# hahnyuan/PTQ4ViT

Measured on AMD Instinct MI355X. Metric: calibration throughput (wrapped modules calibrated per second), ViT-B/224 W8A8, 32 calibration images, higher is better.
Workload: dtype int8

## Files before the change

### include/ptq4vit_hip_debug.h

```cpp
#ifndef PTQ4VIT_HIP_DEBUG_H
#define PTQ4VIT_HIP_DEBUG_H

#include <stdint.h>

#ifdef __cplusplus
extern "C" {
#endif

int p4v_debug_set_variant(int variant, int force_generic);
int p4v_debug_set_tuning(int key, int value);
int p4v_debug_bound_totals(float* out, int64_t capacity, int64_t* count);
int p4v_debug_topk_rows(const float* d_mass, int segs, int n, int k, int32_t* d_idx, void* stream);
int p4v_debug_pack_dual(const float* d_x, long rows, long cols, long cols_padded, int sos, int lo, int hi, int qmax,
                        const float* d_scale, float const_scale, int8_t* d_q1, int8_t* d_q2, void* stream);
int p4v_debug_pack_cands(const float* d_x, long rows, long cols, long rows_padded, long cols_padded, int layout, int lo, int hi,
                         const float* d_scales, int n_cands, const int* d_crange, const unsigned char* d_done, int live_max,
                         int general, int8_t* d_q, void* stream);
int p4v_debug_gather_im2col(int batch, int in_channels, int height, int width, int kernel_h, int kernel_w, int stride_h, int stride_w,
                            int pad_h, int pad_w, int dil_h, int dil_w, const float* d_x, const int32_t* d_idx, int k, float* d_dst,
                            void* stream);
int p4v_debug_prep_epi6(const float* d_o, const float* d_wt, const float* d_bias, long o_ss, long o_ts, int sr, int tr,
                        int bias_on_t, int wt_mode, int transposed, float* d_e, void* stream);

#ifdef __cplusplus
}
#endif
#endif
```

### ptq4vit_amd/_lib.py

```python
import ctypes as C
import os

_HERE = os.path.dirname(os.path.abspath(__file__))
LIB_PATH = os.environ.get("P4V_LIB") or os.path.join(_HERE, "csrc", "libptq4vit_hip.so")

METRICS = {
    "L1_norm": 0,
    "L2_norm": 1,
    "linear_weighted_L2_norm": 2,
    "square_weighted_L2_norm": 3,
    "hessian": 4,
    "cosine": 5,
}


class LinearDesc(C.Structure):
    _fields_ = [(n, C.c_int32) for n in (
        "batch", "tokens", "in_features", "out_features", "n_V", "n_H", "n_a", "w_bit", "a_bit", "metric",
        "eq_n", "search_round", "twin_postgelu", "init_layerwise", "has_bias", "reserved")]


class MatMulDesc(C.Structure):
    _fields_ = ([(n, C.c_int32) for n in ("batch", "heads", "M", "K", "N")] + [("_pad0", C.c_int32)] +
                [("a_stride", C.c_int64 * 4), ("b_stride", C.c_int64 * 4)] +
# ... 43 lines not shown
                ("scale1_stride", C.c_int64 * 4), ("scale1_div", C.c_int32 * 4),
                ("scale2_stride", C.c_int64 * 4), ("scale2_div", C.c_int32 * 4),
                ("scale2_const", C.c_float),
                ("mode", C.c_int32), ("lo1", C.c_int32), ("hi1", C.c_int32), ("lo2", C.c_int32), ("hi2", C.c_int32),
                ("qmax", C.c_int32), ("reserved", C.c_int32)]


class GroupJob(C.Structure):
    _fields_ = [("kind", C.c_int32), ("status", C.c_int32), ("desc", C.c_void_p), ("inp", C.c_void_p * 5), ("mult", C.c_void_p),
                ("out", C.c_void_p * 3), ("workspace", C.c_void_p), ("workspace_bytes", C.c_size_t)]


JOB_LINEAR, JOB_MATMUL, JOB_CONV, JOB_MATMUL_BLOCKS = 0, 1, 2, 3
PLANE_SYM, PLANE_SOS_HI, PLANE_SOS_LO, PLANE_TWIN = 1, 2, 3, 4
EXPORT_SYM_I8, EXPORT_SYM_F32, EXPORT_GELU_U8, EXPORT_SOS_U8 = 0, 1, 2, 3


EXPORTS = [
    "p4v_version", "p4v_last_error",
    "p4v_linear_workspace_bytes", "p4v_linear_calibrate",
    "p4v_matmul_workspace_bytes", "p4v_matmul_calibrate",
    "p4v_matmul_blocks_workspace_bytes", "p4v_matmul_blocks_calibrate", "p4v_amax_init_matmul_blocks",
    "p4v_matmul_blocks_search", "p4v_matmul_blocks_quant_forward",
    "p4v_conv_workspace_bytes", "p4v_conv_calibrate",
    "p4v_calibrate_group", "p4v_launch_counters",
    "p4v_linear_quant_forward", "p4v_matmul_quant_forward",
    "p4v_amax_init_linear", "p4v_linear_search_w", "p4v_linear_search_a",
    "p4v_amax_init_matmul", "p4v_matmul_search_A", "p4v_sos_search_split", "p4v_matmul_search_B",
    "p4v_amax_init_conv", "p4v_conv_search_w_channelwise", "p4v_conv_search_w_layerwise", "p4v_conv_search_a",
    "p4v_score_argmax_gather",
    "p4v_quantize_i8", "p4v_pack_plane_i8", "p4v_fake_quant", "p4v_export_quantize", "p4v_multi_copy",
    "p4v_stats_enable", "p4v_stats_reset", "p4v_stats_get", "p4v_stats_launches", "p4v_prune_counters",
    "p4v_debug_set_variant", "p4v_debug_set_tuning", "p4v_debug_bound_totals", "p4v_debug_topk_rows", "p4v_debug_pack_dual", "p4v_debug_prep_epi6",
    "p4v_debug_pack_cands", "p4v_debug_gather_im2col",
]

_lib = None


def load():
    global _lib
    if _lib is not None:
        return _lib
    if not os.path.exists(LIB_PATH):
        raise RuntimeError(
            f"ptq4vit_amd: HIP extension {LIB_PATH} is missing -- build it with "
            "`python -c 'import __graft_entry__ as g; g.build()'` (hipcc --offload-arch=gfx950). "
            "There is no CPU fallback for the calibration path.")
    import torch
    lib = C.CDLL(LIB_PATH)
    vp, fp, ip = C.c_void_p, C.c_void_p, C.c_void_p
    lib.p4v_version.restype = C.c_int
    lib.p4v_last_error.restype = C.c_char_p
    lib.p4v_linear_workspace_bytes.restype = C.c_size_t
    lib.p4v_linear_workspace_bytes.argtypes = [C.POINTER(LinearDesc)]
    lib.p4v_linear_calibrate.restype = C.c_int
    lib.p4v_linear_calibrate.argtypes = [C.POINTER(LinearDesc), fp, fp, fp, fp, fp, fp, fp, fp, fp, ip, vp, C.c_size_t, vp]
    lib.p4v_matmul_workspace_bytes.restype = C.c_size_t
    lib.p4v_matmul_workspace_bytes.argtypes = [C.POINTER(MatMulDesc)]
    lib.p4v_matmul_calibrate.restype = C.c_int
    lib.p4v_matmul_calibrate.argtypes = [C.POINTER(MatMulDesc), fp, fp, fp, fp, fp, fp, fp, fp, fp, ip, vp, C.c_size_t, vp]
    MBD = C.POINTER(MatMulBlocksDesc)
    lib.p4v_matmul_blocks_workspace_bytes.restype = C.c_size_t
    lib.p4v_matmul_blocks_workspace_bytes.argtypes = [MBD]
    lib.p4v_matmul_blocks_calibrate.restype = C.c_int
    lib.p4v_matmul_blocks_calibrate.argtypes = [MBD, fp, fp, fp, fp, fp, fp, fp, fp, fp, ip, vp, C.c_size_t, vp]
    lib.p4v_amax_init_matmul_blocks.restype = C.c_int
# ... 18 lines not shown
            ("p4v_linear_search_a", [LD] + [fp] * 9 + [ip]),
            ("p4v_amax_init_matmul", [MD] + [fp] * 4),
            ("p4v_matmul_search_A", [MD] + [fp] * 8 + [ip]),
            ("p4v_sos_search_split", [MD] + [fp] * 7 + [ip]),
            ("p4v_matmul_search_B", [MD] + [fp] * 9 + [ip]),
            ("p4v_amax_init_conv", [CD] + [fp] * 4),
            ("p4v_conv_search_w_channelwise", [CD] + [fp] * 9 + [ip]),
            ("p4v_conv_search_w_layerwise", [CD] + [fp] * 9 + [ip]),
            ("p4v_conv_search_a", [CD] + [fp] * 9 + [ip])):
        fn = getattr(lib, name)
        fn.restype = C.c_int
        fn.argtypes = args + tail
    lib.p4v_score_argmax_gather.restype = C.c_int
    lib.p4v_score_argmax_gather.argtypes = [fp, C.c_int32, C.c_int32, fp, fp, ip, vp]
    lib.p4v_quantize_i8.restype = C.c_int
    lib.p4v_quantize_i8.argtypes = [fp, C.c_int64, C.c_int64, C.c_int64, fp, C.c_int64, C.c_int32, C.c_int32, vp, vp]
    lib.p4v_fake_quant.restype = C.c_int
    lib.p4v_fake_quant.argtypes = [fp, C.c_int64, C.c_int64, fp, C.c_int64, C.c_int32, C.c_int32, fp, vp]
    lib.p4v_pack_plane_i8.restype = C.c_int
    lib.p4v_pack_plane_i8.argtypes = [C.POINTER(PlaneDesc), fp, fp, vp, vp]
    lib.p4v_export_quantize.restype = C.c_int
    lib.p4v_export_quantize.argtypes = [C.POINTER(ExportDesc), fp, fp, fp, vp, vp]
    lib.p4v_multi_copy.restype = C.c_int
    lib.p4v_multi_copy.argtypes = [vp, C.c_int32, C.c_int64, C.c_int64, vp]
    lib.p4v_debug_topk_rows.restype = C.c_int
    lib.p4v_debug_topk_rows.argtypes = [vp, C.c_int, C.c_int, C.c_int, vp, vp]
    lib.p4v_debug_pack_dual.restype = C.c_int
    lib.p4v_debug_pack_dual.argtypes = [fp, C.c_long, C.c_long, C.c_long, C.c_int, C.c_int, C.c_int, C.c_int, fp, C.c_float, vp, vp, vp]
    lib.p4v_debug_pack_cands.restype = C.c_int
    lib.p4v_debug_pack_cands.argtypes = [fp, C.c_long, C.c_long, C.c_long, C.c_long, C.c_int, C.c_int, C.c_int, fp, C.c_int, vp, vp,
                                         C.c_int, C.c_int, vp, vp]
    lib.p4v_debug_gather_im2col.restype = C.c_int
    lib.p4v_debug_gather_im2col.argtypes = [C.c_int] * 12 + [fp, ip, C.c_int, fp, vp]
    lib.p4v_debug_prep_epi6.restype = C.c_int
    lib.p4v_debug_prep_epi6.argtypes = [fp, fp, fp, C.c_long, C.c_long, C.c_int, C.c_int, C.c_int, C.c_int, C.c_int, fp, vp]
    lib.p4v_debug_set_variant.restype = C.c_int
    lib.p4v_debug_set_variant.argtypes = [C.c_int, C.c_int]
    lib.p4v_debug_set_tuning.restype = C.c_int
    lib.p4v_debug_set_tuning.argtypes = [C.c_int, C.c_int]
    lib.p4v_debug_bound_totals.restype = C.c_int
    lib.p4v_debug_bound_totals.argtypes = [fp, C.c_int64, C.POINTER(C.c_int64)]
    lib.p4v_stats_enable.restype = C.c_int
    lib.p4v_stats_enable.argtypes = [C.c_int]
    lib.p4v_stats_reset.restype = C.c_int
    lib.p4v_stats_get.restype = C.c_int
    lib.p4v_stats_get.argtypes = [C.POINTER(KernelStats)]
    lib.p4v_stats_launches.restype = C.c_int
    lib.p4v_stats_launches.argtypes = [C.POINTER(LaunchRecord), C.c_int64, C.POINTER(C.c_int64)]
    lib.p4v_prune_counters.restype = C.c_int
    lib.p4v_prune_counters.argtypes = [C.POINTER(C.c_int64), C.c_int]
    lib.p4v_launch_counters.restype = C.c_int
    lib.p4v_launch_counters.argtypes = [C.POINTER(C.c_int64), C.c_int]
    lib.p4v_calibrate_group.restype = C.c_int
    lib.p4v_calibrate_group.argtypes = [C.POINTER(GroupJob), C.c_int32, vp, vp]
    _lib = lib
    return lib


def check(rc, what):
    if rc != 0:
        msg = load().p4v_last_error().decode("utf-8", "replace")
        if rc == -2:
            raise NotImplementedError(f"{what}: {msg}")
        raise RuntimeError(f"{what} failed (code {rc}): {msg}")


# ... 9 lines not shown
```

### ptq4vit_amd/csrc/p4v_api.hip

```cpp
#include <hip/hip_runtime.h>

#include <algorithm>
#include <atomic>
#include <climits>
#include <cstdarg>
#include <cstdio>
#include <condition_variable>
#include <cstring>
#include <deque>
#include <functional>
#include <thread>
#include <mutex>
#include <string>
#include <unordered_map>
#include <type_traits>
#include <vector>

#include "../../include/ptq4vit_hip.h"
#include "../../include/ptq4vit_hip_debug.h"
#include "p4v_kernels.h"

using namespace p4v;

namespace {
// ... 1721 lines not shown
            if (tune(TUNE_PRINT) > 0) fprintf(stderr, "[p4v] second tier: %d survivors of the %d-row slice -> %d of the %d-row slice (M %d N %d K %d)\n", nsurv, k, std::max(0, h[1] - h[0]), k2, ps.Mrows, ps.Ncols, ps.K);
            if (h[0] >= h[1]) return select_without_b2();
            rB = r3; rBblk = rblk3;
            hlo = h[0]; hhi = h[1];
            if (hm && ps.nj <= MIR_BLK) { for (int i = 0; i < 2 * ps.nj; ++i) hblk[i] = reinterpret_cast<volatile int*>(hm)[MIR_RB2 + i]; }
            else hblk_ok = false;
        }
    }
    Pass b2 = ps;
    b2.crange = rB; b2.crange_blk = rBblk; b2.scores_keep = S2; b2.no_select = true;
    b2.host_lo = hlo; b2.host_hi = hhi; b2.host_rblk = hblk_ok ? hblk : nullptr;
    b2.S1_pre = S1s; b2.S2_pre = S2s; b2.s_ready = true;
    g_stage = 3;
    { const int r_ = run_pass(c, b2); g_stage = 0; if (r_) return r_; }
    if (!c.dry) {
        if (virt) CHK(enqueue(c, KERN(MergeVirtParams, k_merge_virtual), dim3(cdiv(ps.nj, 64)), dim3(64), 0, MergeVirtParams{S2, SB, best_idx, ps.nj}));
        else CHK(enqueue(c, KERN(MergeParams, k_merge_scores), dim3(cdiv((long)tab, 256)), dim3(256), 0, MergeParams{S2, SB, (int)tab}));
        CHK(launch_pass_select(c, ps, S2));
    }
    c.ws.off = mark;
    return 0;
}

struct SosSplitJob {
    SliceCache* scache; bool host_sync_ok, prunable;
    SosSplitParams kp;
    int epi; double norm;
    const float* cands; float* split; float* A_iv; float aux_div;
    float* scores_out; int scores_out_ld; int32_t* best_out;
};
bool sos_split_ok(int M, int K, int N, bool cosm) {
    return !cosm && K <= 200 && M <= 256 && N <= 64 && !(g_variant & 131072);
}
template <int KS> int launch_sos_split_ks(Ctx& c, const SosSplitParams& kp, int epi, const StatInfo* si) {
    const dim3 grid(kp.halves, kp.Z), block(256);
    const size_t lds = (size_t)2 * KS * 64 * sizeof(float);
    P4V_EPI4(epi, return enqueue(c, KERN_T(SosSplitParams, k_sos_split, KS, E), grid, block, lds, kp, si))
}
SelectParams sos_select_params(const SosSplitJob& j, const float* scores) {
    return SelectParams{scores, j.kp.C, 1, j.cands, 1, 0, 0, j.split, 0, 0, j.A_iv, j.aux_div, j.scores_out, j.scores_out_ld, j.best_out};
}
int sos_sweep(Ctx& c, SosSplitJob& j, SosSplitParams kp, const int* crange, float* scores, int known_cands = -1) {
    const int slots = kp.halves * 4;
    float* part = c.ws.get<float>((size_t)kp.C * kp.Z * slots);
    if (!c.ws.ok()) return fail(P4V_ERR_WORKSPACE, "workspace too small: need >= %zu bytes", c.ws.off);
    kp.part = part; kp.crange = crange;
    if (!c.dry) {
        CHK(q_fill(c, part, 0, sizeof(float) * (size_t)kp.C * kp.Z * slots));
        const int KS = kp.K <= 64 ? 32 : kp.K <= 144 ? 72 : 100;
        double frac = 1.0;
        if (g_stat_on && crange && known_cands >= 0) frac = (double)known_cands / kp.C;
        else if (g_stat_on && crange) {
            int h[2] = {0, kp.C};
            CHK(q_d2h(c, h, crange, sizeof h));
            CHK(q_sync(c));
            frac = (double)std::max(0, std::min(h[1], kp.C) - std::max(h[0], 0)) / kp.C;
        }
        const StatInfo si{11, frac * (double)kp.Z * kp.halves * 128 * (2.0 * KS) * 64 * kp.C, frac * (double)kp.Z * kp.M * kp.K * kp.N * kp.C, g_stage, kp.halves, kp.Z,
                          4.0 * ((double)kp.Z * kp.M * kp.K + (double)kp.Z * kp.K * kp.N) + 8.0 * (double)kp.Z * kp.M * kp.N};
        const StatInfo* sp = &si;
        if (KS == 32) CHK(launch_sos_split_ks<32>(c, kp, j.epi, sp));
        else if (KS == 72) CHK(launch_sos_split_ks<72>(c, kp, j.epi, sp));
        else CHK(launch_sos_split_ks<100>(c, kp, j.epi, sp));
    }
    FinishParams fp{part, (long)kp.Z * slots, (long)slots, slots, 1, kp.Z, slots, kp.C, 0, 1, 1, j.norm, scores, crange};
    return launch_finish(c, fp);
}
int sos_select(Ctx& c, SosSplitJob& j, const float* scores) {
    return launch_select(c, sos_select_params(j, scores));
}
int run_sos_split(Ctx& c, SosSplitJob& j) {
    const size_t mark = c.ws.off;
    float* scores = c.ws.get<float>((size_t)j.kp.C);
    CHK(sos_sweep(c, j, j.kp, nullptr, scores));
    CHK(sos_select(c, j, scores));
    c.ws.off = mark;
    return 0;
}
int run_sos_split_pruned_impl(Ctx& c, SosSplitJob& j);
int run_sos_split_pruned(Ctx& c, SosSplitJob& j) {
    if (!(g_variant & 134217728) || c.dry || !j.split) return run_sos_split_pruned_impl(c, j);
    std::vector<float> keep;
    CHK(run_sos_split_pruned_impl(c, j));
    CHK(prune_crosscheck_begin(c, j.split, 1, keep));
    CHK(run_sos_split(c, j));
    return prune_crosscheck_end(c, j.split, 1, keep, "split search");
}
int run_sos_split_pruned_impl(Ctx& c, SosSplitJob& j) {
    const SosSplitParams& kp = j.kp;
    const int k = 16;
    if (!j.prunable || !j.scache || j.scores_out || j.best_out || (g_variant & 4194304) || kp.M < 64 || j.scache->loose) {
        PRUNE_COUNT((!j.prunable || !j.scache || j.scores_out || j.best_out || (g_variant & 4194304)) ? 3 : 2);
        return run_sos_split(c, j);
    }
    SliceGeo geo{false, kp.Z, kp.M, k, kp.N, kp.K, kp.O, (kp.wt_mode == 1 ? kp.G : nullptr), kp.wt_mode, (long)kp.N, kp.A, kp.a_r, kp.a_k,
                 kp.zdiv, kp.a_z2, kp.a_z, false, PackParams{}, k};
    SliceCache* sc = j.scache;
    CHK(slice_alloc(c, sc, geo, true, false));
    const size_t mark = c.ws.off;
// ... 503 lines not shown
            }
        }
        if (skip_A || !(sg.mask & ST_S1)) {
        } else if (!d->sos) {
            Pass ps{};
            common(ps);
            ps.i8 = true; ps.twin = false; ps.eq_n = d->eq_n;
            Operand a = A_operand(true, A_cands, H, PACK_SYM), b = B_operand(false, B_iv, 0, PACK_SYM);
            if (!cosm) { ps.row = a; ps.col = b; } else { ps.row = b; ps.col = a; }
            ps.use_s1 = true; ps.s_cs = H; ps.sb_mode = 2; ps.sb_div = H;
            ps.s1 = ScaleParams{A_cands, H, 1, 0.f, B_iv, 0, 1, 0.f, 0, 0, nullptr};
            ps.j_mode = 2; ps.j_div = H; ps.nj = H; ps.cos_j_mode = 2; ps.cos_j_div = H;
            ps.norm = cosm ? 1.0 / (double)M : 1.0 / ((double)M * N);
            ps.cands = A_cands; ps.cand_cs = H; ps.cand_js = 1; ps.interval = A_iv; ps.out_js = 1;
            ps.cache = keep_planes ? &plane_A : nullptr;
            ps.scores_out = so; ps.scores_out_ld = H; ps.best_out = bo;
            ps.prunable = !cosm && !(d->reserved & 8); ps.scache = &slice; ps.host_sync_ok = memo_on;
            CHK(run_pass_pruned(c, ps));
        } else if (sos_split_ok(M, K, N, cosm)) {
            SosSplitJob j{};
            j.kp.A = A; j.kp.a_z2 = d->a_stride[0]; j.kp.a_z = d->a_stride[1]; j.kp.a_r = d->a_stride[2]; j.kp.a_k = d->a_stride[3];
            j.kp.zdiv = H;
            j.kp.B = B; j.kp.b_z2 = d->b_stride[0]; j.kp.b_z = d->b_stride[1]; j.kp.b_k = d->b_stride[2]; j.kp.b_n = d->b_stride[3];
            j.kp.O = O; j.kp.G = G ? G : O;
            j.kp.Z = Z; j.kp.M = M; j.kp.K = K; j.kp.N = N; j.kp.wt_mode = wt_mode; j.kp.C = NSPLIT;
            j.kp.splits = split_cands;
            j.kp.qm1 = (float)(Aq - 1); j.kp.c_inv = 1.0f / (float)(Aq - 1);
            j.kp.lo_top = std::min(std::nearbyintf(1.0f / j.kp.c_inv), (float)(Aq - 1));
            j.kp.halves = cdiv(M, 128);
            j.epi = epi; j.norm = 1.0 / ((double)H * M * N);
            j.cands = split_cands; j.split = split; j.A_iv = A_iv; j.aux_div = (float)(Aq - 1);
            j.scores_out = (d->eq_n >= NSPLIT) ? so : nullptr; j.scores_out_ld = H; j.best_out = bo;
            j.scache = &slice; j.host_sync_ok = memo_on; j.prunable = !(d->reserved & 8);
            CHK(run_sos_split_pruned(c, j));
        } else {
            Pass ps{};
            common(ps);
            ps.i8 = false; ps.twin = false; ps.eq_n = NSPLIT;
            Operand a = A_operand(true, split_cands, 1, PACK_SOS_SIM), b = B_operand(false, nullptr, 0, PACK_RAW);
            if (!cosm) { ps.row = a; ps.col = b; } else { ps.row = b; ps.col = a; }
            ps.use_s1 = false; ps.s_cs = 1; ps.sb_mode = 0;
            ps.j_mode = 0; ps.nj = 1; ps.cos_j_mode = 0;
            ps.norm = cosm ? 1.0 / ((double)H * M) : 1.0 / ((double)H * M * N);
            ps.cands = split_cands; ps.cand_cs = 1; ps.cand_js = 0; ps.interval = split; ps.out_js = 0;
            ps.aux_out = A_iv; ps.aux_div = (float)(Aq - 1);
            ps.scores_out = (d->eq_n >= NSPLIT) ? so : nullptr; ps.scores_out_ld = H; ps.best_out = bo;
            CHK(run_pass(c, ps));
        }
        if (memo_on && !skip_A) {
            if (d->sos) { std::vector<float> sp, ai; CHK(read_dev(c, split, 1, sp)); CHK(read_dev(c, A_iv, 1, ai)); val = {sp[0], ai[0]}; }
            else CHK(read_dev(c, A_iv, nAiv, val));
            memo_A.entries.push_back({key, val}); g_memo_misses++;
        }
        bool skip_B = false;
        if (memo_on) {
            CHK(read_dev(c, A_iv, nAiv, key));
            if (const auto* hit = memo_B.find(key)) { CHK(write_dev(c, B_iv, *hit)); skip_B = true; g_memo_hits++; }
        }
        if (!skip_B && (sg.mask & ST_S2)) {
            Pass ps{};
            common(ps);
            ps.eq_n = d->eq_n;
            const bool twin_rows = d->sos && !cosm;
            ps.i8 = !(d->sos && cosm);
            ps.twin = twin_rows;
            Operand b = B_operand(true, B_cands, H, PACK_SYM);
// ... 811 lines not shown

int p4v_stats_launches(p4v_launch_record* out, int64_t capacity, int64_t* count) {
    int r = stats_drain();
    if (r) return r;
    if (count) *count = (int64_t)g_stat_done.size();
    if (out)
        for (int64_t i = 0; i < capacity && i < (int64_t)g_stat_done.size(); ++i) {
            const StatRec& s = g_stat_done[(size_t)i];
            out[i] = p4v_launch_record{s.kind, s.stage, s.gx, s.gz, (double)s.ms, 2.0 * s.macs, 2.0 * s.alg, s.bytes};
        }
    return 0;
}

int p4v_prune_counters(int64_t* out4, int reset) {
    if (out4) for (int i = 0; i < 4; ++i) out4[i] = (int64_t)g_prune_cnt[i].load(std::memory_order_relaxed);
    if (reset) for (int i = 0; i < 4; ++i) g_prune_cnt[i].store(0, std::memory_order_relaxed);
    return 0;
}

int p4v_debug_set_variant(int variant, int force_generic) {
    if (variant < 0 || variant >= (1 << 30)) return fail(P4V_ERR_INVALID, "p4v_debug_set_variant: bad variant word");
    if (variant & ~VARIANT_KEPT) return fail(P4V_ERR_INVALID, "p4v_debug_set_variant: bits 0x%x select removed paths", variant & ~VARIANT_KEPT);
    g_variant_word.store(variant | (force_generic ? (1 << 30) : 0), std::memory_order_relaxed);
    return 0;
}

int p4v_debug_set_tuning(int key, int value) {
    if (key < 0 || key >= 16) return fail(P4V_ERR_INVALID, "p4v_debug_set_tuning: unknown key %d", key);
    if (key == TUNE_B1_PATH && tune_b1_removed(value)) return fail(P4V_ERR_INVALID, "p4v_debug_set_tuning: 12 = %d selects a removed path", value);
    g_tune[key].store(value, std::memory_order_relaxed);
    return 0;
}

int p4v_debug_bound_totals(float* out, int64_t capacity, int64_t* count) {
    if (!out && !count) { g_b1_keep = true; g_b1_totals.clear(); return 0; }
    g_b1_keep = false;
    if (count) *count = (int64_t)g_b1_totals.size();
    if (out) std::copy(g_b1_totals.begin(), g_b1_totals.begin() + std::min<int64_t>(capacity, (int64_t)g_b1_totals.size()), out);
    return 0;
}

int p4v_debug_topk_rows(const float* d_mass, int segs, int n, int k, int32_t* d_idx, void* stream) {
    if (!d_mass || !d_idx || segs <= 0 || n <= 0 || k <= 0 || k > n) return fail(P4V_ERR_INVALID, "p4v_debug_topk_rows: bad argument");
    hipLaunchKernelGGL(k_topk_rows, dim3(segs), dim3(1024), 0, (hipStream_t)stream, TopkParams{d_mass, n, k, d_idx});
    HIPCHK(hipGetLastError());
    return 0;
}

int p4v_debug_pack_dual(const float* d_x, long rows, long cols, long cols_padded, int sos, int lo, int hi, int qmax,
                        const float* d_scale, float const_scale, int8_t* d_q1, int8_t* d_q2, void* stream) {
    if (!d_x || !d_scale || !d_q1 || !d_q2 || rows <= 0 || cols <= 0 || cols_padded % 64 || cols_padded < cols ||
        lo > 0 || hi < 0 || lo < -128 || hi > 127 || qmax < 2 || qmax > 128 || (!sos && !(const_scale > 0.0f)))
        return fail(P4V_ERR_INVALID, "p4v_debug_pack_dual: bad argument");
    PackParams p1 = pack2d(d_x, rows, cols, cols);
    p1.Rp = (int)rows; p1.Kp = (int)cols_padded; p1.C = 1; p1.scales = d_scale; p1.qm1 = (float)(qmax - 1);
    PackParams p2 = p1;
    p1.dst = d_q1; p2.dst = d_q2;
    if (sos) {
        p1.mode = PACK_SOS_HI; p2.mode = PACK_SOS_LO;
    } else {
        p1.lo = 0; p1.hi = hi; p2.lo = lo; p2.hi = 0; p2.scales = nullptr; p2.neg_scale = const_scale;
    }
    if (!dual_pack_ok(p1, p2)) return fail(P4V_ERR_INVALID, "p4v_debug_pack_dual: not a dual pair");
    Ctx c{(hipStream_t)stream, Arena(nullptr, 0), false};
    const long total = rows * (cols_padded / 16);
    if (total >= (1L << 31)) return fail(P4V_ERR_UNSUPPORTED, "p4v_debug_pack_dual: plane too large");
// ... 111 lines not shown
```

### ptq4vit_amd/csrc/p4v_kernels.h

```cpp
#pragma once
#include <hip/hip_runtime.h>
#include <stdint.h>
#include <type_traits>

namespace p4v {

typedef int v4i __attribute__((ext_vector_type(4)));
typedef int v16i __attribute__((ext_vector_type(16)));
typedef float v4f __attribute__((ext_vector_type(4)));
typedef float v16f __attribute__((ext_vector_type(16)));
typedef float v2f __attribute__((ext_vector_type(2)));

#ifndef P4V_GROUP_KERNARG
#define P4V_GROUP_KERNARG (4096 - 256)
#endif
template <typename P> struct GroupArgs {
    static constexpr int CAP_RAW = (P4V_GROUP_KERNARG - 16) / (int)(sizeof(P) + 16);
    static constexpr int CAP = CAP_RAW > 64 ? 64 : CAP_RAW;
    int n;
    unsigned off[CAP + 1];
    unsigned gx[CAP], gy[CAP], gz[CAP];
    P p[CAP];
};
#define P4V_BIDX uint3{blockIdx.x, blockIdx.y, blockIdx.z}
// ... 3092 lines not shown
                first(it + 1, std::integral_constant<int, 1>{}); second(it + 1, std::integral_constant<int, 1>{}); __builtin_amdgcn_s_barrier();
                first(it + 2, std::integral_constant<int, 2>{}); second(it + 2, std::integral_constant<int, 2>{}); __builtin_amdgcn_s_barrier();
                first(it + 3, std::integral_constant<int, 3>{}); second(it + 3, std::integral_constant<int, 3>{});
                if (kq + 4 < ktiles) __builtin_amdgcn_s_barrier();
            }
            if constexpr (!(P4V_SW7_DBG & 4)) epilogue(ci);
            __builtin_amdgcn_s_barrier();
        }
    }
#undef P4V_DSR
#undef P4V_GLD
    __syncthreads();
    if constexpr (COS) return;
    for (int i = tid; i < ncand * 32; i += 512) {
        const int cc = c_lo + (i >> 5), wv = (i >> 2) & 7, j = i & 3;
        p.part[(long)cc * p.p_cs + (long)(ct * 4 + (wv & 3)) * p.NG + rt * 8 + (wv >> 2) * 4 + j] = res[i];
    }
}
template <int TW, int EPI>
__global__ __launch_bounds__(512, 2) void k_sweep7(Sweep7Params p) { k_sweep7_body<TW, EPI>(p, P4V_BIDX, P4V_GDIM); }
template <int TW, int EPI>
__global__ __launch_bounds__(512, 2) void k_sweep7_g(GroupArgs<Sweep7Params> a) { P4V_GROUP_ENTER(a); k_sweep7_body<TW, EPI>(a.p[m_], vb_, vg_); }

struct SosSplitParams {
    const float* A; long a_z2, a_z, a_r, a_k; int zdiv;
    const float* B; long b_z2, b_z, b_k, b_n;
    const float* O; const float* G;
    int Z, M, K, N, wt_mode, C;
    const float* splits;
    float qm1, c_inv, lo_top;
    float* part;
    int halves;
    const int* crange;
};

#ifndef P4V_SOS_DBG
#define P4V_SOS_DBG 0
#endif
template <int KS, int EPI>
__device__ __forceinline__ void k_sos_split_body(const SosSplitParams& p, const uint3 blockIdx, const uint3 gridDim) {
    extern __shared__ __attribute__((aligned(16))) char smem[];
    float* Bt = reinterpret_cast<float*>(smem);
    const int tid = threadIdx.x, lane = tid & 63;
    const int wid = __builtin_amdgcn_readfirstlane(tid >> 6);
    const int g = lane >> 5, l31 = lane & 31;
    const int half = blockIdx.x, z = blockIdx.y;
    const long zoffA = p.zdiv > 0 ? (long)(z / p.zdiv) * p.a_z2 + (long)(z % p.zdiv) * p.a_z : (long)z * p.a_z;
    const long zoffB = p.zdiv > 0 ? (long)(z / p.zdiv) * p.b_z2 + (long)(z % p.zdiv) * p.b_z : (long)z * p.b_z;

    for (int i = tid; i < 2 * KS * 64; i += 256) {
        const int k = i >> 6, n = i & 63;
        Bt[i] = (k < p.K && n < p.N) ? p.B[zoffB + (long)k * p.b_k + (long)n * p.b_n] : 0.0f;
    }
    const bool share = p.M <= 32 && p.halves == 1;
    const int row0 = share ? 0 : half * 128 + wid * 32;
    const int row = row0 + l31;
    float hv[KS], yv[KS];
    {
        const float* ap = p.A + zoffA + (long)min(row, p.M - 1) * p.a_r;
#pragma unroll
        for (int ks = 0; ks < KS; ++ks) {
            const int k = 2 * ks + g;
            const float x = (row < p.M && k < p.K) ? ap[(long)k * p.a_k] : 0.0f;
            hv[ks] = rintf(x * p.qm1) / p.qm1;
            yv[ks] = x / p.c_inv;
        }
    }
    float u[2][16], w[2][16];
#pragma unroll
    for (int cb = 0; cb < 2; ++cb)
#pragma unroll
        for (int r = 0; r < 16; ++r) {
            const int m = row0 + (r & 3) + 8 * (r >> 2) + 4 * g, n = cb * 32 + l31;
            const bool ok = m < p.M && n < p.N;
            const long idx = ((long)z * p.M + min(m, p.M - 1)) * p.N + min(n, p.N - 1);
            const float o = p.O[idx];
            const float gw = p.wt_mode == 1 ? p.G[idx] : p.wt_mode == 2 ? o : p.wt_mode == 3 ? fabsf(o) : 1.0f;
            u[cb][r] = ok ? o : 0.0f;
            w[cb][r] = ok ? gw : 0.0f;
        }
    __syncthreads();
    if (row0 >= p.M) return;

    typedef float v16f __attribute__((ext_vector_type(16)));
    const float* b0 = Bt + g * 64 + l31;
    int c_lo_ = 0, c_hi_ = p.C;
    clip_crange(p.crange, c_lo_, c_hi_);
    for (int c = c_lo_ + (share ? wid : 0); c < c_hi_; c += share ? 4 : 1) {
        const float s = p.splits[c];
        const float inv_s = 1.0f / s;
        const float a_int = s / p.qm1;
        const float cl = rintf(s * p.qm1) / p.qm1;
        v16f acc0 = {0, 0, 0, 0, 0, 0, 0, 0, 0, 0, 0, 0, 0, 0, 0, 0}, acc1 = acc0;
        float bq0[3], bq1[3], aq[3];
        auto stage = [&](auto ks_c) __attribute__((always_inline)) {
            constexpr int ks = decltype(ks_c)::value;
            if constexpr (ks < KS) {
                if constexpr ((P4V_SOS_DBG & 2) != 0) { bq0[ks % 3] = cl; bq1[ks % 3] = inv_s; }
                else { bq0[ks % 3] = b0[ks * 128]; bq1[ks % 3] = b0[ks * 128 + 32]; }
                if constexpr ((P4V_SOS_DBG & 1) != 0) { aq[ks % 3] = hv[ks] + yv[ks]; return; }
                const float hi = __builtin_amdgcn_fmed3f(hv[ks], cl, 1.0f);
                const float li = __builtin_amdgcn_fmed3f(rintf(yv[ks] * inv_s), 0.0f, p.lo_top);
                float lo = li * a_int;
                asm volatile("" : "+v"(lo));
                aq[ks % 3] = hi + lo;
            }
        };
        stage(std::integral_constant<int, 0>{});
        stage(std::integral_constant<int, 1>{});
        [&]<int... S>(std::integer_sequence<int, S...>) __attribute__((always_inline)) {
            ([&] {
                stage(std::integral_constant<int, S + 2>{});
                if constexpr ((P4V_SOS_DBG & 4) != 0) { acc0[S % 16] += aq[S % 3] * bq0[S % 3]; acc1[S % 16] += aq[S % 3] * bq1[S % 3]; }
                else {
                    acc0 = __builtin_amdgcn_mfma_f32_32x32x2f32(aq[S % 3], bq0[S % 3], acc0, 0, 0, 0);
                    acc1 = __builtin_amdgcn_mfma_f32_32x32x2f32(aq[S % 3], bq1[S % 3], acc1, 0, 0, 0);
                }
                __builtin_amdgcn_sched_barrier(0);
            }(), ...);
        }(std::make_integer_sequence<int, KS>{});
        float sum = 0.0f;
#pragma unroll
        for (int cb = 0; cb < 2; ++cb)
#pragma unroll
            for (int r = 0; r < 16; ++r) {
                const float d = u[cb][r] - (cb ? acc1[r] : acc0[r]);
                const float ww = w[cb][r];
                if (EPI == EPI_SQ_W) { const float t2 = ww * d; sum = fmaf(t2, t2, sum); }
                else if (EPI == EPI_SQ) sum = fmaf(ww * d, d, sum);
                else if (EPI == EPI_ABS) sum = fmaf(ww, fabsf(d), sum);
                else sum = fmaf(ww * d, d, sum);
            }
        sum = wave_sum_dpp(sum);
        if (lane == 63) p.part[((long)c * p.Z + z) * (p.halves * 4) + half * 4 + wid] = sum;
    }
}
template <int KS, int EPI>
__global__ __launch_bounds__(256, 1) void k_sos_split(SosSplitParams p) { k_sos_split_body<KS, EPI>(p, P4V_BIDX, P4V_GDIM); }
template <int KS, int EPI>
__global__ __launch_bounds__(256, 1) void k_sos_split_g(GroupArgs<SosSplitParams> a) { P4V_GROUP_ENTER(a); k_sos_split_body<KS, EPI>(a.p[m_], vb_, vg_); }

__device__ __forceinline__ bool score_beats(float av, int ai, float bv, int bi) {
    const bool an = av != av, bn = bv != bv;
    if (an != bn) return an;
    if (an) return ai < bi;
    return av > bv || (av == bv && ai < bi);
}
__device__ __forceinline__ int block_argmax(float v, int i, float* sv, int* si) {
    const int t = threadIdx.x;
    sv[t] = v; si[t] = i;
    __syncthreads();
    for (int o = blockDim.x >> 1; o > 0; o >>= 1) {
        if (t < o && score_beats(sv[t + o], si[t + o], sv[t], si[t])) { sv[t] = sv[t + o]; si[t] = si[t + o]; }
        __syncthreads();
    }
    const int r = si[0];
    __syncthreads();
    return r;
}

struct SelectParams {
    const float* scores; int C, nj;
    const float* cands; int cand_cs, cand_js, cand_off;
    float* interval; int out_js, out_off;
    float* aux_out; float aux_div;
    float* scores_out;
    int scores_out_ld;
    int32_t* best_out;
    float* iv_host; float* aux_host;
};
__device__ __forceinline__ void select_block(const SelectParams& p, int j, int c_lo, int c_hi, float* sv, int* si) {
    float bv = -__builtin_inff();
    int bi = 0x7fffffff;
// ... 795 lines not shown
```

### ptq4vit_amd/engine.py

```python
import ctypes as C

import torch

from . import _lib

_workspace = {}
_mult_cache = {}


def _require_cuda(t, what):
    if not t.is_cuda:
        raise RuntimeError(f"ptq4vit_amd: {what} must live on the GPU (got {t.device}); the calibration path has no CPU fallback")


def device_of(*tensors):
    for t in tensors:
        if t is not None and t.is_cuda:
            return t.device
    if not torch.cuda.is_available():
        raise RuntimeError("ptq4vit_amd: no GPU visible -- the HIP calibration engine needs an MI355X (no CPU fallback)")
    return torch.device("cuda", torch.cuda.current_device())


def to_dev(t, dev):
# ... 657 lines not shown
                                              ptr(crange) if crange is not None else None,
                                              ptr(done) if done is not None else None, int(live_max), int(bool(general)),
                                              ptr(out), stream_ptr(x2d.device))
    _lib.check(rc, "p4v_debug_pack_cands")
    return out


def debug_gather_im2col(x, idx, *, kernel_size, stride, padding, dilation):
    assert x.is_cuda and x.dtype == torch.float32 and x.dim() == 4 and idx.is_cuda and idx.dtype == torch.int32 and idx.dim() == 1
    x, idx = x.contiguous(), idx.contiguous()
    b, ic, H, W = x.shape
    (kh, kw), (sh, sw), (ph, pw), (dh, dw) = kernel_size, stride, padding, dilation
    fh, fw = (H + 2 * ph - dh * (kh - 1) - 1) // sh + 1, (W + 2 * pw - dw * (kw - 1) - 1) // sw + 1
    if fh > 0 and fw > 0:
        assert idx.numel() > 0 and int(idx.min()) >= 0 and int(idx.max()) < b * fh * fw, "row index outside the im2col matrix"
    out = torch.full((idx.numel(), ic * kh * kw), float("nan"), dtype=torch.float32, device=x.device)
    with torch.cuda.device(x.device):
        rc = _lib.load().p4v_debug_gather_im2col(b, ic, H, W, kh, kw, sh, sw, ph, pw, dh, dw, ptr(x), ptr(idx), idx.numel(), ptr(out),
                                                 stream_ptr(x.device))
    _lib.check(rc, "p4v_debug_gather_im2col")
    return out


def debug_prep_epi6(o, wt, bias, *, o_ss, o_ts, sr, tr, bias_on_t, wt_mode, transposed):
    n = -(-sr // 256) * -(-tr // 64) * 256 * 64 * 2
    e = torch.full((n,), float("nan"), dtype=torch.float32, device=o.device)
    with torch.cuda.device(o.device):
        rc = _lib.load().p4v_debug_prep_epi6(ptr(o), ptr(wt) if wt is not None else None, ptr(bias), int(o_ss), int(o_ts),
                                             int(sr), int(tr), int(bias_on_t), int(wt_mode), int(transposed), ptr(e),
                                             stream_ptr(o.device))
    _lib.check(rc, "p4v_debug_prep_epi6")
    return e

def stats_reset():
    _lib.load().p4v_stats_reset()


def stats_get():
    s = _lib.KernelStats()
    _lib.check(_lib.load().p4v_stats_get(C.byref(s)), "p4v_stats_get")
    return {k: getattr(s, k) for k, _ in _lib.KernelStats._fields_}


def prune_counters(reset=False):
    out = (C.c_int64 * 4)()
    _lib.check(_lib.load().p4v_prune_counters(out, int(bool(reset))), "p4v_prune_counters")
    return dict(zip(("staged", "staged_no_survivors", "kept_full_sweep", "not_eligible"), (int(v) for v in out)))


def stats_launches():
    lib = _lib.load()
    n = C.c_int64(0)
    _lib.check(lib.p4v_stats_launches(None, 0, C.byref(n)), "p4v_stats_launches")
    buf = (_lib.LaunchRecord * max(1, n.value))()
    _lib.check(lib.p4v_stats_launches(buf, n.value, C.byref(n)), "p4v_stats_launches")
    return [{"kernel": _lib.LAUNCH_KINDS.get(r.kind, str(r.kind)), "stage": _lib.LAUNCH_STAGES.get(r.stage, str(r.stage)),
             "grid_x": r.grid_x, "grid_z": r.grid_z, "ms": r.ms, "ops": r.ops, "alg_ops": r.alg_ops, "alg_bytes": r.alg_bytes}
            for r in buf[:n.value]]
```

Measured before the change: 672.3.

## Add specialized split-of-softmax search kernel variants with vectorized B staging

Splits the split-of-softmax search kernel into variants picked by shape and known candidate count. A pair variant handles two candidates per wave for very small M. A light variant recomputes the A-side quantized images per candidate instead of holding them in registers, which allows two blocks per CU. The loads now use vectorized float4 B staging into LDS and 32-bit offset addressing, with global loads issued early and kept apart by scheduling barriers. A debug entry point for sweeping candidates is also added, at the cost of more template instantiations and extra recomputation in the light path.

Measured after the change: 694.2 (median of 6 runs). 1.03x the previous value.

```diff
diff --git a/include/ptq4vit_hip_debug.h b/include/ptq4vit_hip_debug.h
--- a/include/ptq4vit_hip_debug.h
+++ b/include/ptq4vit_hip_debug.h
@@ -10,6 +10,9 @@
 int p4v_debug_set_variant(int variant, int force_generic);
 int p4v_debug_set_tuning(int key, int value);
 int p4v_debug_bound_totals(float* out, int64_t capacity, int64_t* count);
+int p4v_debug_sos_sweep(const p4v_matmul_desc* desc, const float* d_A, const float* d_B, const float* d_out, const float* d_grad,
+                        int n_cands, int c_lo, int c_hi, int known_cands, float* d_scores, void* d_workspace, size_t workspace_bytes,
+                        void* stream);
 int p4v_debug_topk_rows(const float* d_mass, int segs, int n, int k, int32_t* d_idx, void* stream);
 int p4v_debug_pack_dual(const float* d_x, long rows, long cols, long cols_padded, int sos, int lo, int hi, int qmax,
                         const float* d_scale, float const_scale, int8_t* d_q1, int8_t* d_q2, void* stream);
diff --git a/ptq4vit_amd/_lib.py b/ptq4vit_amd/_lib.py
--- a/ptq4vit_amd/_lib.py
+++ b/ptq4vit_amd/_lib.py
@@ -99,7 +99,7 @@
     "p4v_quantize_i8", "p4v_pack_plane_i8", "p4v_fake_quant", "p4v_export_quantize", "p4v_multi_copy",
     "p4v_stats_enable", "p4v_stats_reset", "p4v_stats_get", "p4v_stats_launches", "p4v_prune_counters",
     "p4v_debug_set_variant", "p4v_debug_set_tuning", "p4v_debug_bound_totals", "p4v_debug_topk_rows", "p4v_debug_pack_dual", "p4v_debug_prep_epi6",
-    "p4v_debug_pack_cands", "p4v_debug_gather_im2col",
+    "p4v_debug_pack_cands", "p4v_debug_gather_im2col", "p4v_debug_sos_sweep",
 ]
 
 _lib = None
@@ -184,6 +184,8 @@
                                          C.c_int, C.c_int, vp, vp]
     lib.p4v_debug_gather_im2col.restype = C.c_int
     lib.p4v_debug_gather_im2col.argtypes = [C.c_int] * 12 + [fp, ip, C.c_int, fp, vp]
+    lib.p4v_debug_sos_sweep.restype = C.c_int
+    lib.p4v_debug_sos_sweep.argtypes = [C.POINTER(MatMulDesc), fp, fp, fp, fp, C.c_int, C.c_int, C.c_int, C.c_int, fp, vp, C.c_size_t, vp]
     lib.p4v_debug_prep_epi6.restype = C.c_int
     lib.p4v_debug_prep_epi6.argtypes = [fp, fp, fp, C.c_long, C.c_long, C.c_int, C.c_int, C.c_int, C.c_int, C.c_int, fp, vp]
     lib.p4v_debug_set_variant.restype = C.c_int
diff --git a/ptq4vit_amd/csrc/p4v_api.hip b/ptq4vit_amd/csrc/p4v_api.hip
--- a/ptq4vit_amd/csrc/p4v_api.hip
+++ b/ptq4vit_amd/csrc/p4v_api.hip
@@ -1777,10 +1777,32 @@
 bool sos_split_ok(int M, int K, int N, bool cosm) {
     return !cosm && K <= 200 && M <= 256 && N <= 64 && !(g_variant & 131072);
 }
-template <int KS> int launch_sos_split_ks(Ctx& c, const SosSplitParams& kp, int epi, const StatInfo* si) {
+template <int KS, int VAR> int launch_sos_split_var(Ctx& c, const SosSplitParams& kp, int epi, const StatInfo* si) {
     const dim3 grid(kp.halves, kp.Z), block(256);
     const size_t lds = (size_t)2 * KS * 64 * sizeof(float);
-    P4V_EPI4(epi, return enqueue(c, KERN_T(SosSplitParams, k_sos_split, KS, E), grid, block, lds, kp, si))
+    P4V_EPI4(epi, return enqueue(c, KERN_T(SosSplitParams, k_sos_split, KS, E, VAR), grid, block, lds, kp, si))
+}
+template <int KS> int launch_sos_split_ks(Ctx& c, const SosSplitParams& kp, int var, int epi, const StatInfo* si) {
+    switch (var) {
+        case SOS_PREV: return launch_sos_split_var<KS, SOS_PREV>(c, kp, epi, si);
+        case SOS_PAIR: return launch_sos_split_var<KS, SOS_PAIR>(c, kp, epi, si);
+        case SOS_LIGHT: return launch_sos_split_var<KS, SOS_LIGHT>(c, kp, epi, si);
+        default: return launch_sos_split_var<KS, SOS_RES>(c, kp, epi, si);
+    }
+}
+constexpr int SOS_LIGHT_MAX = 2;
+int sos_variant(const SosSplitParams& kp, int known_cands) {
+    const int path = tune(TUNE_B1_PATH);
+    if (path == 13) return SOS_PREV;
+    if (kp.halves == 1 && kp.M <= 16) return SOS_PAIR;
+    if (kp.halves == 1 && kp.M <= 32) return SOS_RES;
+    const bool a_compact = kp.a_r >= 0 && kp.a_k >= 0 && ((long)(kp.M - 1) * kp.a_r + (long)(kp.K - 1) * kp.a_k) * 4 < (1L << 31);
+    if (path != 14 && a_compact && known_cands >= 1 && (known_cands <= SOS_LIGHT_MAX || path == 15)) return SOS_LIGHT;
+    return SOS_RES;
+}
+bool sos_b_vector_ok(const SosSplitParams& kp) {
+    return kp.b_n == 1 && kp.N % 4 == 0 && reinterpret_cast<uintptr_t>(kp.B) % 16 == 0 && kp.b_k % 4 == 0 && kp.b_z % 4 == 0 &&
+           (kp.zdiv <= 0 || kp.b_z2 % 4 == 0);
 }
 SelectParams sos_select_params(const SosSplitJob& j, const float* scores) {
     return SelectParams{scores, j.kp.C, 1, j.cands, 1, 0, 0, j.split, 0, 0, j.A_iv, j.aux_div, j.scores_out, j.scores_out_ld, j.best_out};
@@ -1790,6 +1812,7 @@
     float* part = c.ws.get<float>((size_t)kp.C * kp.Z * slots);
     if (!c.ws.ok()) return fail(P4V_ERR_WORKSPACE, "workspace too small: need >= %zu bytes", c.ws.off);
     kp.part = part; kp.crange = crange;
+    kp.bvec = sos_b_vector_ok(kp) ? 1 : 0;
     if (!c.dry) {
         CHK(q_fill(c, part, 0, sizeof(float) * (size_t)kp.C * kp.Z * slots));
         const int KS = kp.K <= 64 ? 32 : kp.K <= 144 ? 72 : 100;
@@ -1804,12 +1827,31 @@
         const StatInfo si{11, frac * (double)kp.Z * kp.halves * 128 * (2.0 * KS) * 64 * kp.C, frac * (double)kp.Z * kp.M * kp.K * kp.N * kp.C, g_stage, kp.halves, kp.Z,
                           4.0 * ((double)kp.Z * kp.M * kp.K + (double)kp.Z * kp.K * kp.N) + 8.0 * (double)kp.Z * kp.M * kp.N};
         const StatInfo* sp = &si;
-        if (KS == 32) CHK(launch_sos_split_ks<32>(c, kp, j.epi, sp));
-        else if (KS == 72) CHK(launch_sos_split_ks<72>(c, kp, j.epi, sp));
-        else CHK(launch_sos_split_ks<100>(c, kp, j.epi, sp));
+        const int var = sos_variant(kp, crange ? known_cands : -1);
+        if (KS == 32) CHK(launch_sos_split_ks<32>(c, kp, var, j.epi, sp));
+        else if (KS == 72) CHK(launch_sos_split_ks<72>(c, kp, var, j.epi, sp));
+        else CHK(launch_sos_split_ks<100>(c, kp, var, j.epi, sp));
     }
     FinishParams fp{part, (long)kp.Z * slots, (long)slots, slots, 1, kp.Z, slots, kp.C, 0, 1, 1, j.norm, scores, crange};
     return launch_finish(c, fp);
+}
+struct SosDebugSweep { int n_cands, c_lo, c_hi, known_cands; float* d_scores; };
+thread_local const SosDebugSweep* g_sos_debug = nullptr;
+int run_sos_debug_sweep(Ctx& c, SosSplitJob& j, const SosDebugSweep& dbg) {
+    const size_t mark = c.ws.off;
+    SosSplitParams kp = j.kp;
+    kp.C = dbg.n_cands;
+    float* scores = c.ws.get<float>((size_t)kp.C);
+    int* r = c.ws.get<int>(2);
+    if (!c.ws.ok()) return fail(P4V_ERR_WORKSPACE, "workspace too small: need >= %zu bytes", c.ws.off);
+    const int h[2] = {dbg.c_lo, dbg.c_hi};
+    const bool ranged = dbg.c_lo >= 0;
+    if (ranged) { CHK(q_h2d(c, r, h, sizeof h)); CHK(q_sync(c)); }
+    CHK(sos_sweep(c, j, kp, ranged ? r : nullptr, scores, dbg.known_cands));
+    HIPCHK(hipMemcpyAsync(dbg.d_scores, scores, sizeof(float) * (size_t)kp.C, hipMemcpyDeviceToDevice, c.st));
+    CHK(q_sync(c));
+    c.ws.off = mark;
+    return 0;
 }
 int sos_select(Ctx& c, SosSplitJob& j, const float* scores) {
     return launch_select(c, sos_select_params(j, scores));
@@ -2379,6 +2421,7 @@
             j.cands = split_cands; j.split = split; j.A_iv = A_iv; j.aux_div = (float)(Aq - 1);
             j.scores_out = (d->eq_n >= NSPLIT) ? so : nullptr; j.scores_out_ld = H; j.best_out = bo;
             j.scache = &slice; j.host_sync_ok = memo_on; j.prunable = !(d->reserved & 8);
+            if (g_sos_debug) return c.grp || c.dry ? fail(P4V_ERR_INVALID, "p4v_debug_sos_sweep: not inside a group") : run_sos_debug_sweep(c, j, *g_sos_debug);
             CHK(run_sos_split_pruned(c, j));
         } else {
             Pass ps{};
@@ -3256,6 +3299,24 @@
     return 0;
 }
 
+int p4v_debug_sos_sweep(const p4v_matmul_desc* desc, const float* d_A, const float* d_B, const float* d_out, const float* d_grad,
+                        int n_cands, int c_lo, int c_hi, int known_cands, float* d_scores, void* d_workspace, size_t workspace_bytes,
+                        void* stream) {
+    if (!desc || !d_A || !d_B || !d_out || !d_scores || !d_workspace) return fail(P4V_ERR_INVALID, "p4v_debug_sos_sweep: null pointer");
+    if (!desc->sos || n_cands < 1 || n_cands > 20 || !sos_split_ok(desc->M, desc->K, desc->N, false))
+        return fail(P4V_ERR_INVALID, "p4v_debug_sos_sweep: a split-of-softmax matmul of the one-kernel split search, 1..20 candidates");
+    const SosDebugSweep dbg{n_cands, c_lo, c_hi, known_cands, d_scores};
+    float* d_split = nullptr;
+    HIPCHK(hipMalloc(&d_split, 2 * sizeof(float)));
+    Ctx c{(hipStream_t)stream, Arena(d_workspace, workspace_bytes), false};
+    g_sos_debug = &dbg;
+    const int rc = matmul_impl(desc, d_A, d_B, d_out, d_grad, nullptr, d_split + 1, nullptr, d_split, nullptr, nullptr, c, nullptr,
+                               Stage{ST_S1, nullptr, nullptr});
+    g_sos_debug = nullptr;
+    (void)hipFree(d_split);
+    return rc;
+}
+
 int p4v_debug_bound_totals(float* out, int64_t capacity, int64_t* count) {
     if (!out && !count) { g_b1_keep = true; g_b1_totals.clear(); return 0; }
     g_b1_keep = false;
diff --git a/ptq4vit_amd/csrc/p4v_kernels.h b/ptq4vit_amd/csrc/p4v_kernels.h
--- a/ptq4vit_amd/csrc/p4v_kernels.h
+++ b/ptq4vit_amd/csrc/p4v_kernels.h
@@ -3148,53 +3148,147 @@
     float* part;
     int halves;
     const int* crange;
+    int bvec;
 };
 
 #ifndef P4V_SOS_DBG
 #define P4V_SOS_DBG 0
 #endif
-template <int KS, int EPI>
+enum { SOS_PREV = 0, SOS_RES = 1, SOS_PAIR = 2, SOS_LIGHT = 3 };
+template <int KS, int EPI, int VAR>
 __device__ __forceinline__ void k_sos_split_body(const SosSplitParams& p, const uint3 blockIdx, const uint3 gridDim) {
     extern __shared__ __attribute__((aligned(16))) char smem[];
     float* Bt = reinterpret_cast<float*>(smem);
+    constexpr bool PAIR = VAR == SOS_PAIR, LIGHT = VAR == SOS_LIGHT;
+    constexpr int NR = PAIR ? 8 : 16;
     const int tid = threadIdx.x, lane = tid & 63;
     const int wid = __builtin_amdgcn_readfirstlane(tid >> 6);
     const int g = lane >> 5, l31 = lane & 31;
     const int half = blockIdx.x, z = blockIdx.y;
     const long zoffA = p.zdiv > 0 ? (long)(z / p.zdiv) * p.a_z2 + (long)(z % p.zdiv) * p.a_z : (long)z * p.a_z;
     const long zoffB = p.zdiv > 0 ? (long)(z / p.zdiv) * p.b_z2 + (long)(z % p.zdiv) * p.b_z : (long)z * p.b_z;
-
-    for (int i = tid; i < 2 * KS * 64; i += 256) {
-        const int k = i >> 6, n = i & 63;
-        Bt[i] = (k < p.K && n < p.N) ? p.B[zoffB + (long)k * p.b_k + (long)n * p.b_n] : 0.0f;
-    }
-    const bool share = p.M <= 32 && p.halves == 1;
+    const bool share = PAIR || (p.M <= 32 && p.halves == 1);
     const int row0 = share ? 0 : half * 128 + wid * 32;
-    const int row = row0 + l31;
-    float hv[KS], yv[KS];
-    {
-        const float* ap = p.A + zoffA + (long)min(row, p.M - 1) * p.a_r;
-#pragma unroll
-        for (int ks = 0; ks < KS; ++ks) {
-            const int k = 2 * ks + g;
-            const float x = (row < p.M && k < p.K) ? ap[(long)k * p.a_k] : 0.0f;
-            hv[ks] = rintf(x * p.qm1) / p.qm1;
-            yv[ks] = x / p.c_inv;
-        }
-    }
-    float u[2][16], w[2][16];
-#pragma unroll
-    for (int cb = 0; cb < 2; ++cb)
-#pragma unroll
-        for (int r = 0; r < 16; ++r) {
-            const int m = row0 + (r & 3) + 8 * (r >> 2) + 4 * g, n = cb * 32 + l31;
-            const bool ok = m < p.M && n < p.N;
-            const long idx = ((long)z * p.M + min(m, p.M - 1)) * p.N + min(n, p.N - 1);
-            const float o = p.O[idx];
-            const float gw = p.wt_mode == 1 ? p.G[idx] : p.wt_mode == 2 ? o : p.wt_mode == 3 ? fabsf(o) : 1.0f;
-            u[cb][r] = ok ? o : 0.0f;
-            w[cb][r] = ok ? gw : 0.0f;
-        }
+    const int row = row0 + (PAIR ? (l31 & 15) : l31);
+    float hv[LIGHT ? 1 : KS], yv[LIGHT ? 1 : KS], xr[KS];
+    float u[2][NR], w[2][NR];
+    auto images = [&](auto ks_c) __attribute__((always_inline)) {
+        constexpr int ks = decltype(ks_c)::value;
+        hv[ks] = rintf(xr[ks] * p.qm1) / p.qm1;
+        yv[ks] = xr[ks] / p.c_inv;
+    };
+    if constexpr (VAR == SOS_PREV) {
+        for (int i = tid; i < 2 * KS * 64; i += 256) {
+            const int k = i >> 6, n = i & 63;
+            Bt[i] = (k < p.K && n < p.N) ? p.B[zoffB + (long)k * p.b_k + (long)n * p.b_n] : 0.0f;
+        }
+        {
+            const float* ap = p.A + zoffA + (long)min(row, p.M - 1) * p.a_r;
+#pragma unroll
+            for (int ks = 0; ks < KS; ++ks) {
+                const int k = 2 * ks + g;
+                const float x = (row < p.M && k < p.K) ? ap[(long)k * p.a_k] : 0.0f;
+                hv[ks] = rintf(x * p.qm1) / p.qm1;
+                yv[ks] = x / p.c_inv;
+            }
+        }
+#pragma unroll
+        for (int cb = 0; cb < 2; ++cb)
+#pragma unroll
+            for (int r = 0; r < 16; ++r) {
+                const int m = row0 + (r & 3) + 8 * (r >> 2) + 4 * g, n = cb * 32 + l31;
+                const bool ok = m < p.M && n < p.N;
+                const long idx = ((long)z * p.M + min(m, p.M - 1)) * p.N + min(n, p.N - 1);
+                const float o = p.O[idx];
+                const float gw = p.wt_mode == 1 ? p.G[idx] : p.wt_mode == 2 ? o : p.wt_mode == 3 ? fabsf(o) : 1.0f;
+                u[cb][r] = ok ? o : 0.0f;
+                w[cb][r] = ok ? gw : 0.0f;
+            }
+    } else {
+        const float* bp = p.B + zoffB;
+        auto load_a = [&]() __attribute__((always_inline)) {
+            if constexpr (LIGHT) {
+                const char* ab = reinterpret_cast<const char*>(p.A + zoffA);
+                const unsigned ro = (unsigned)min(row, p.M - 1) * (unsigned)p.a_r, ak = (unsigned)p.a_k;
+#pragma unroll
+                for (int ks = 0; ks < KS; ++ks)
+                    xr[ks] = *reinterpret_cast<const float*>(ab + (size_t)((ro + (unsigned)min(2 * ks + g, p.K - 1) * ak) * 4u));
+            } else {
+                const float* ap = p.A + zoffA + (long)min(row, p.M - 1) * p.a_r;
+#pragma unroll
+                for (int ks = 0; ks < KS; ++ks)
+                    xr[ks] = ap[(long)min(2 * ks + g, p.K - 1) * p.a_k];
+            }
+        };
+        auto load_og = [&]() __attribute__((always_inline)) {
+            const char* ob = reinterpret_cast<const char*>(p.O + (long)z * p.M * p.N);
+            const char* gb = reinterpret_cast<const char*>(p.G + (long)z * p.M * p.N);
+#pragma unroll
+            for (int cb = 0; cb < 2; ++cb)
+#pragma unroll
+                for (int r = 0; r < NR; ++r) {
+                    const int m = row0 + (r & 3) + 8 * (r >> 2) + 4 * g, n = cb * 32 + l31;
+                    u[cb][r] = *reinterpret_cast<const float*>(ob + (size_t)((unsigned)(min(m, p.M - 1) * p.N + min(n, p.N - 1)) * 4u));
+                }
+            if (p.wt_mode == 1) {
+#pragma unroll
+                for (int cb = 0; cb < 2; ++cb)
+#pragma unroll
+                    for (int r = 0; r < NR; ++r) {
+                        const int m = row0 + (r & 3) + 8 * (r >> 2) + 4 * g, n = cb * 32 + l31;
+                        w[cb][r] = *reinterpret_cast<const float*>(gb + (size_t)((unsigned)(min(m, p.M - 1) * p.N + min(n, p.N - 1)) * 4u));
+                    }
+            }
+        };
+        auto loads = [&](auto vec_c) __attribute__((always_inline)) {
+            constexpr bool VEC = decltype(vec_c)::value;
+            constexpr int W = VEC ? 4 : 1;
+            constexpr int NB = (2 * KS * 64 / W + 255) / 256;
+            typedef float piece __attribute__((ext_vector_type(W)));
+            piece bb[NB];
+#pragma unroll
+            for (int t = 0; t < NB; ++t) {
+                const int i = (tid + t * 256) * W, k = i >> 6, n = i & 63;
+                bb[t] = *reinterpret_cast<const piece*>(bp + (long)min(k, p.K - 1) * p.b_k + (VEC ? (long)min(n, p.N - 4) : (long)min(n, p.N - 1) * p.b_n));
+            }
+            if constexpr (!LIGHT) { load_a(); load_og(); }
+            __builtin_amdgcn_sched_barrier(0);
+#pragma unroll
+            for (int t = 0; t < NB; ++t) {
+                const int i = (tid + t * 256) * W, k = i >> 6, n = i & 63;
+                const piece v = (k < p.K && n < p.N) ? bb[t] : piece(0.0f);
+                if (NB * 256 * W == 2 * KS * 64 || i < 2 * KS * 64) *reinterpret_cast<piece*>(Bt + i) = v;
+            }
+            if constexpr (LIGHT) { __builtin_amdgcn_sched_barrier(0); load_a(); load_og(); __builtin_amdgcn_sched_barrier(0); }
+        };
+        if (p.bvec) loads(std::true_type{}); else loads(std::false_type{});
+        const int kg = row < p.M ? p.K - g : 0;
+#pragma unroll
+        for (int ks = 0; ks < KS; ++ks) xr[ks] = 2 * ks < kg ? xr[ks] : 0.0f;
+        if constexpr (!LIGHT) {
+            [&]<int... S>(std::integer_sequence<int, S...>) __attribute__((always_inline)) {
+                (images(std::integral_constant<int, S>{}), ...);
+            }(std::make_integer_sequence<int, KS>{});
+        }
+        auto weights = [&](auto wsel_c) __attribute__((always_inline)) {
+            constexpr int wsel = decltype(wsel_c)::value;
+#pragma unroll
+          for (int cb = 0; cb < 2; ++cb)
+#pragma unroll
+            for (int r = 0; r < NR; ++r) {
+                const int m = row0 + (r & 3) + 8 * (r >> 2) + 4 * g, n = cb * 32 + l31;
+                const bool ok = m < p.M && n < p.N;
+                const float o = u[cb][r];
+                const float gw = wsel == 0 ? w[cb][r] : wsel == 1 ? o : wsel == 2 ? fabsf(o) : 1.0f;
+                u[cb][r] = ok ? o : 0.0f;
+                w[cb][r] = ok ? gw : 0.0f;
+            }
+        };
+        if (p.wt_mode == 1) weights(std::integral_constant<int, 0>{});
+        else if (p.wt_mode == 2) weights(std::integral_constant<int, 1>{});
+        else if (p.wt_mode == 3) weights(std::integral_constant<int, 2>{});
+        else weights(std::integral_constant<int, 3>{});
+    }
     __syncthreads();
     if (row0 >= p.M) return;
 
@@ -3202,8 +3296,10 @@
     const float* b0 = Bt + g * 64 + l31;
     int c_lo_ = 0, c_hi_ = p.C;
     clip_crange(p.crange, c_lo_, c_hi_);
-    for (int c = c_lo_ + (share ? wid : 0); c < c_hi_; c += share ? 4 : 1) {
-        const float s = p.splits[c];
+    constexpr int CW = PAIR ? 2 : 1;
+    for (int c = c_lo_ + (share ? wid * CW : 0); c < c_hi_; c += share ? 4 * CW : CW) {
+        const bool two = PAIR && c + 1 < c_hi_;
+        const float s = (PAIR && two && (l31 & 16)) ? p.splits[c + 1] : p.splits[c];
         const float inv_s = 1.0f / s;
         const float a_int = s / p.qm1;
         const float cl = rintf(s * p.qm1) / p.qm1;
@@ -3214,9 +3310,16 @@
             if constexpr (ks < KS) {
                 if constexpr ((P4V_SOS_DBG & 2) != 0) { bq0[ks % 3] = cl; bq1[ks % 3] = inv_s; }
                 else { bq0[ks % 3] = b0[ks * 128]; bq1[ks % 3] = b0[ks * 128 + 32]; }
-                if constexpr ((P4V_SOS_DBG & 1) != 0) { aq[ks % 3] = hv[ks] + yv[ks]; return; }
-                const float hi = __builtin_amdgcn_fmed3f(hv[ks], cl, 1.0f);
-                const float li = __builtin_amdgcn_fmed3f(rintf(yv[ks] * inv_s), 0.0f, p.lo_top);
+                float hvk, yvk;
+                if constexpr (LIGHT) {
+                    float x = xr[ks];
+                    asm volatile("" : "+v"(x));
+                    hvk = rintf(x * p.qm1) / p.qm1;
+                    yvk = x / p.c_inv;
+                } else { hvk = hv[ks]; yvk = yv[ks]; }
+                if constexpr ((P4V_SOS_DBG & 1) != 0) { aq[ks % 3] = hvk + yvk; return; }
+                const float hi = __builtin_amdgcn_fmed3f(hvk, cl, 1.0f);
+                const float li = __builtin_amdgcn_fmed3f(rintf(yvk * inv_s), 0.0f, p.lo_top);
                 float lo = li * a_int;
                 asm volatile("" : "+v"(lo));
                 aq[ks % 3] = hi + lo;
@@ -3235,26 +3338,30 @@
                 __builtin_amdgcn_sched_barrier(0);
             }(), ...);
         }(std::make_integer_sequence<int, KS>{});
-        float sum = 0.0f;
-#pragma unroll
-        for (int cb = 0; cb < 2; ++cb)
-#pragma unroll
-            for (int r = 0; r < 16; ++r) {
-                const float d = u[cb][r] - (cb ? acc1[r] : acc0[r]);
-                const float ww = w[cb][r];
-                if (EPI == EPI_SQ_W) { const float t2 = ww * d; sum = fmaf(t2, t2, sum); }
-                else if (EPI == EPI_SQ) sum = fmaf(ww * d, d, sum);
-                else if (EPI == EPI_ABS) sum = fmaf(ww, fabsf(d), sum);
-                else sum = fmaf(ww * d, d, sum);
-            }
-        sum = wave_sum_dpp(sum);
-        if (lane == 63) p.part[((long)c * p.Z + z) * (p.halves * 4) + half * 4 + wid] = sum;
-    }
-}
-template <int KS, int EPI>
-__global__ __launch_bounds__(256, 1) void k_sos_split(SosSplitParams p) { k_sos_split_body<KS, EPI>(p, P4V_BIDX, P4V_GDIM); }
-template <int KS, int EPI>
-__global__ __launch_bounds__(256, 1) void k_sos_split_g(GroupArgs<SosSplitParams> a) { P4V_GROUP_ENTER(a); k_sos_split_body<KS, EPI>(a.p[m_], vb_, vg_); }
+#pragma unroll
+        for (int h = 0; h < CW; ++h) {
+            float sum = 0.0f;
+#pragma unroll
+            for (int cb = 0; cb < 2; ++cb)
+#pragma unroll
+                for (int r = 0; r < NR; ++r) {
+                    const float d = u[cb][r] - (cb ? acc1[h * NR + r] : acc0[h * NR + r]);
+                    const float ww = w[cb][r];
+                    if (EPI == EPI_SQ_W) { const float t2 = ww * d; sum = fmaf(t2, t2, sum); }
+                    else if (EPI == EPI_SQ) sum = fmaf(ww * d, d, sum);
+                    else if (EPI == EPI_ABS) sum = fmaf(ww, fabsf(d), sum);
+                    else sum = fmaf(ww * d, d, sum);
+                }
+            sum = wave_sum_dpp(sum);
+            const int slot = PAIR ? ((c + h - c_lo_) & 3) : wid;
+            if (lane == 63 && (h == 0 || two)) p.part[((long)(c + h) * p.Z + z) * (p.halves * 4) + half * 4 + slot] = sum;
+        }
+    }
+}
+template <int KS, int EPI, int VAR>
+__global__ __launch_bounds__(256, VAR == SOS_LIGHT ? 2 : 1) void k_sos_split(SosSplitParams p) { k_sos_split_body<KS, EPI, VAR>(p, P4V_BIDX, P4V_GDIM); }
+template <int KS, int EPI, int VAR>
+__global__ __launch_bounds__(256, VAR == SOS_LIGHT ? 2 : 1) void k_sos_split_g(GroupArgs<SosSplitParams> a) { P4V_GROUP_ENTER(a); k_sos_split_body<KS, EPI, VAR>(a.p[m_], vb_, vg_); }
 
 __device__ __forceinline__ bool score_beats(float av, int ai, float bv, int bi) {
     const bool an = av != av, bn = bv != bv;
diff --git a/ptq4vit_amd/engine.py b/ptq4vit_amd/engine.py
--- a/ptq4vit_amd/engine.py
+++ b/ptq4vit_amd/engine.py
@@ -713,6 +713,23 @@
     _lib.check(rc, "p4v_debug_prep_epi6")
     return e
 
+def debug_sos_sweep(*, A, B, out, grad, A_bit, metric, crange=None, known_cands=-1, n_cands=20):
+    lib = _lib.load()
+    dev = device_of(A, B)
+    A, B = to_dev(A, dev), to_dev(B, dev)
+    out = to_dev(out, dev).contiguous()
+    grad = to_dev(grad, dev).contiguous() if grad is not None else None
+    d = _matmul_desc(A, B, A_bit, 8, metric, 100, 1, True, 0, 0)[1]
+    ws = workspace(dev, _need(lib.p4v_matmul_workspace_bytes, d, "p4v_matmul_workspace_bytes"))
+    scores = torch.full((int(n_cands),), float("nan"), dtype=torch.float32, device=dev)
+    lo, hi = (-1, -1) if crange is None else (int(crange[0]), int(crange[1]))
+    with torch.cuda.device(dev):
+        rc = lib.p4v_debug_sos_sweep(C.byref(d), ptr(A), ptr(B), ptr(out), ptr(grad), int(n_cands), lo, hi, int(known_cands),
+                                     ptr(scores), ptr(ws), ws.numel(), stream_ptr(dev))
+    _lib.check(rc, "p4v_debug_sos_sweep")
+    return scores
+
+
 def stats_reset():
     _lib.load().p4v_stats_reset()
 
```
